# agussomacal/ROMHighContrast

Hardware: AMD Instinct MI355X
Metric: snapshot_solves_per_sec (higher is better)
Workload: dtype f64

## Files before the change

romhighcontrast_amd/csrc/rom_fem_kernels.hip:

```cpp
#include "rom_fem_dev.h"

__global__ void k_build_A0(double* A0, const double* Qp, const double* rho, int n1, int n1p, int N) {
  size_t idx = blockIdx.x * size_t(blockDim.x) + threadIdx.x;
  size_t total = size_t(n1) * n1 * n1p;
  if (idx >= total) return;
  int m = int(idx % n1p);
  size_t ij = idx / n1p;
  int j = int(ij % n1) + 1, i = int(ij / n1) + 1;
  A0[idx] = (m < n1) ? Qp[size_t(j - 1) * n1p + m] * rho[size_t(m) * (N + 1) + i] : 0.0;
}

__global__ void k_repack_table(const double* __restrict__ G, int ld, int nseg, int n1, int orient, double* __restrict__ Gs) {
  const long long idx = blockIdx.x * (long long)blockDim.x + threadIdx.x;
  const long long hrows = (long long)n1 * n1;
  if (idx >= (long long)nseg * hrows * 8) return;
  const int kk = int(idx & 7);
  const long long rp = (idx >> 3) % hrows, seg = (idx >> 3) / hrows;
  const long long row = orient ? (rp % n1) * n1 + rp / n1 : rp;
  const int k = int(seg) * 8 + kk;
  Gs[idx] = k < ld ? G[row * ld + k] : 0.0;
}

__global__ void k_mask_table(double* __restrict__ G, int ld, int n1, ExtThresholds th) {
  const long long idx = blockIdx.x * (long long)blockDim.x + threadIdx.x;
// ... 442 lines not shown
  for (int i = threadIdx.x; i < f.nsc; i += blockDim.x) {
    const int b0 = f.scb[2 * i], b1 = f.scb[2 * i + 1];
    y[f.spos0 + i] = b1 >= 0 ? 1.0 / (am[b0] + am[b1]) : (1.0 / (double(f.N) * double(f.N))) / am[b0];
  }
  for (int task = threadIdx.x; task < f.nctask; task += blockDim.x) {
    const int4 t0 = reinterpret_cast<const int4*>(f.ctask)[2 * task], t1 = reinterpret_cast<const int4*>(f.ctask)[2 * task + 1];
    const int len = t0.z, ldm = t0.w;
    const double* Mt = f.cm + t0.x;
    const double* src = ys + t0.y;
    double dot = 0.0;
#pragma unroll 16
    for (int j = 0; j < len; ++j) dot += Mt[size_t(j) * ldm] * src[j];
    if (t1.x >= 0) dot += f.vec[t1.x] / (am[t1.y] + am[t1.z]);
    dots[t1.w] = dot;
  }
  __syncthreads();
  for (int it = threadIdx.x; it < f.ncoef; it += blockDim.x) {
    const CoefGroup& cg = f.groups[f.item_group[it]];
    const int k = f.item_k[it];
    const double s = am[cg.b0] + am[cg.b1];
    double out = 0.0;
    if (k == cg.r) {
      out = 1.0 / s;
    } else if (k < cg.r) {
      if (cg.kind == 0) {
        out = ys[cg.zpos + k];
      } else {
        const double* dk = dots + size_t(f.item_cf[it]) * 8;
        double acc = 0.0;
        for (int t = 0; t < cg.nterm; ++t) acc += (cg.t[t].blk >= 0 ? am[cg.t[t].blk] : s / 2) * dk[t];
        out = acc / s;
      }
    }
    y[cg.cpos + k] = out;
  }
}

__global__ __launch_bounds__(256) void k_expand(FemDev f, const double* __restrict__ a, int Mc, double* __restrict__ U,
                                                long long row0) {
  __shared__ __align__(16) double lds[STAGE_TOTAL];
  expand_tile(f, Mc, U, row0, lds, blockIdx.x, blockIdx.y, blockIdx.z);
}

__global__ __launch_bounds__(256) void k_back_pre(FemDev f, const double* __restrict__ a, int Mc) {
  __shared__ __align__(16) double lds[STAGE_TOTAL];
  const WavePos wp;
  const PreEdge& pe = f.pre[blockIdx.z];
  const int srow = stage_row(), sseg = stage_seg();
  const int mA = blockIdx.y * 64 + srow;
  const int iB = blockIdx.x * 64 + srow;
  const double* am = mA < Mc ? a + size_t(mA) * f.kblk : nullptr;
  const double seA = am ? am[pe.e0] + am[pe.e1] : 0.0;
  Acc acc;
  acc_zero(acc);
  for (int q = 0; q < pe.nnb; ++q) {
    const PreNb nb = pe.nb[q];
    const double* pA = am ? f.y + size_t(mA) * f.nGp + nb.fpos + sseg : nullptr;
    const double* pB = f.Bt + (size_t(nb.bt) * f.n1p + iB) * f.n1p + sseg;
    const double cu = !am ? 0.0 : (nb.blk >= 0 ? am[nb.blk] : seA / 2);
    gemm_loop(
        nb.nch,
        [&](int ch, double* v) {
          load4_aligned(pA ? pA + ch * BK : nullptr, v);
#pragma unroll
          for (int x = 0; x < 4; ++x) v[x] *= cu;
        },
        [&](int ch, double* v) { load4_aligned(pB + ch * BK, v); }, acc, lds, wp);
  }
#pragma unroll
  for (int i = 0; i < 2; ++i)
#pragma unroll
    for (int g = 0; g < 4; ++g) {
      const int m = blockIdx.y * 64 + acc_row(wp, i, g);
      if (m >= Mc) continue;
      const double* amr = a + size_t(m) * f.kblk;
      const double inv = 1.0 / (amr[pe.e0] + amr[pe.e1]);
#pragma unroll
      for (int jb = 0; jb < 2; ++jb) {
        const int node = blockIdx.x * 64 + acc_col(wp, jb);
        f.y[size_t(m) * f.nGp + pe.pos + node] = node < f.n1 ? (f.vec[pe.woff + node] + acc.c[i][jb][g]) * inv : 0.0;
      }
    }
}

template <int NS>
__device__ inline void diag_update_body(const FemDev& f, const double* __restrict__ am0, int m0, int nsys, int slot, double* lds,
                                        double* coef) {
  const WavePos wp;
  const TileDesc& d = f.desc[slot];
  const bool lower = !(wp.wr == 0 && wp.wc == 1);
  if (f.tile_stream && d.t1 - d.t0 <= 128) {
    TileStream<NS> ts;
    s_tile_stream_begin<NS>(ts, slot, d, f, am0, nsys);
    SymAcc acc[NS];
#pragma unroll
    for (int q = 0; q < NS; ++q) {
      sym_acc_zero(acc[q]);
      if (q >= nsys) continue;
      if (q > 0) __syncthreads();
      accumulate_klist_dma<true>(f, slot, f.L + size_t(m0 + q) * f.nslots * 4096, [](int) { return true; }, acc[q], reinterpret_cast<char*>(lds), wp);
    }
    __syncthreads();
    double* T[NS];
#pragma unroll
    for (int q = 0; q < NS; ++q) T[q] = lds + q * TILE_DOUBLES;
    s_tile_to_lds<NS>(T, ts, d, f);
#pragma unroll
    for (int q = 0; q < NS; ++q) {
      if (q >= nsys) break;
      tile_minus_acc_sym(T[q], acc[q], wp);
      double* Lout = f.L + (size_t(m0 + q) * f.nslots + slot) * 4096;
      for (int idx = threadIdx.x; idx < 4096; idx += 256) Lout[idx] = T[q][(idx >> 6) * LDC + (idx & 63)];
    }
    return;
  }
  double* Cb = lds;
  STile st[NS];
  s_tile_load<NS>(st, d, f, am0, nsys, coef);
#pragma unroll
  for (int q = 0; q < NS; ++q) {
    if (q >= nsys) break;
    double* Lm = f.L + size_t(m0 + q) * f.nslots * 4096;
    Acc acc;
    acc_zero(acc);
    if (q > 0) __syncthreads();
    accumulate_klist_dma(f, slot, Lm, [&](int) { return lower; }, acc, reinterpret_cast<char*>(lds), wp);
    tile_from_acc(Cb, acc, st[q], wp);
    double* Lout = Lm + size_t(slot) * 4096;
    for (int idx = threadIdx.x; idx < 4096; idx += 256) Lout[idx] = Cb[(idx >> 6) * LDC + (idx & 63)];
  }
}
template <int NS>
__global__ __launch_bounds__(256, NS == 1 ? 4 : 2) void k_diag_update(FemDev f, const double* __restrict__ a, int slot, int Mc) {
  __shared__ __align__(16) double lds[NS * TILE_DOUBLES];
  __shared__ double coef[NS * COEF_MAX + TERM_DESC_DOUBLES];
  static_assert(TD_LDS_BYTES <= TILE_DOUBLES * 8, "the DMA slots fit under the tile");
  const int m0 = blockIdx.x * NS;
  diag_update_body<NS>(f, a + size_t(m0) * f.kblk, m0, min(NS, Mc - m0), slot, lds, coef);
}
template __global__ void k_diag_update<1>(FemDev, const double*, int, int);
template __global__ void k_diag_update<2>(FemDev, const double*, int, int);

__device__ inline double rsqrt_newton(double d) {
  double y = __builtin_amdgcn_rsq(d);
  const double hd = 0.5 * d;
  y = y * fma(-hd * y, y, 1.5);
  y = y * fma(-hd * y, y, 1.5);
  return y;
}


__device__ __host__ constexpr int s1_lrow(int r) { return 8 * (r >> 2) * ((r >> 2) + 1) + (r & 3) * 4 * ((r >> 2) + 1); }

__device__ inline bool chol_pivots_bad(double myrs) {
  return __builtin_amdgcn_ballot_w64(!(myrs > 0.0 && myrs < 1.0e300)) != 0;
}
__device__ inline void chol_panel_core(int lane, int c0, double (&v)[4], double& y, double& myrs, double a00, double a10,
                                       double a11, double a20, double a21, double a22, double a30, double a31, double a32, double a33) {
  const double y0 = readlane_f64(y, c0);
  double y1 = readlane_f64(y, c0 + 1), y2 = readlane_f64(y, c0 + 2), y3 = readlane_f64(y, c0 + 3);
  const double rs0 = rsqrt_newton(a00);
  const double l10 = a10 * rs0, l20 = a20 * rs0, l30 = a30 * rs0;
  a11 -= l10 * l10; a21 -= l20 * l10; a31 -= l30 * l10;
  a22 -= l20 * l20; a32 -= l30 * l20; a33 -= l30 * l30;
  const double yd0 = y0 * rs0;
  y1 -= l10 * yd0; y2 -= l20 * yd0; y3 -= l30 * yd0;
  {
    const double l = lane >= c0 ? v[0] * rs0 : 0.0;
    v[0] = l;
    if (lane == c0) {
      y = yd0;
      myrs = rs0;
    } else if (lane > c0) {
      y -= l * yd0;
    }
    v[1] -= l * l10; v[2] -= l * l20; v[3] -= l * l30;
  }
  const double rs1 = rsqrt_newton(a11);
  const double l21 = a21 * rs1, l31 = a31 * rs1;
  a22 -= l21 * l21; a32 -= l31 * l21; a33 -= l31 * l31;
  const double yd1 = y1 * rs1;
  y2 -= l21 * yd1; y3 -= l31 * yd1;
  {
    const double l = lane >= c0 + 1 ? v[1] * rs1 : 0.0;
    v[1] = l;
    if (lane == c0 + 1) {
      y = yd1;
      myrs = rs1;
    } else if (lane > c0 + 1) {
      y -= l * yd1;
    }
    v[2] -= l * l21; v[3] -= l * l31;
  }
  const double rs2 = rsqrt_newton(a22);
  const double l32 = a32 * rs2;
  a33 -= l32 * l32;
  const double yd2 = y2 * rs2;
  y3 -= l32 * yd2;
  {
    const double l = lane >= c0 + 2 ? v[2] * rs2 : 0.0;
    v[2] = l;
    if (lane == c0 + 2) {
      y = yd2;
      myrs = rs2;
    } else if (lane > c0 + 2) {
      y -= l * yd2;
    }
    v[3] -= l * l32;
  }
  const double rs3 = rsqrt_newton(a33);
  const double yd3 = y3 * rs3;
  {
    const double l = lane >= c0 + 3 ? v[3] * rs3 : 0.0;
    v[3] = l;
    if (lane == c0 + 3) {
      y = yd3;
      myrs = rs3;
    } else if (lane > c0 + 3) {
      y -= l * yd3;
    }
  }
}
__device__ inline void chol_panel_rows(const double* Pn, int lane, int c0, double (&v)[4], double& y, double& myrs) {
  {
    const double2 v01 = *reinterpret_cast<const double2*>(&Pn[lane * 4]);
    const double2 v23 = *reinterpret_cast<const double2*>(&Pn[lane * 4 + 2]);
    v[0] = v01.x; v[1] = v01.y; v[2] = v23.x; v[3] = v23.y;
  }
  const double a00 = Pn[c0 * 4];
  const double2 r1 = *reinterpret_cast<const double2*>(&Pn[(c0 + 1) * 4]);
  const double2 r2 = *reinterpret_cast<const double2*>(&Pn[(c0 + 2) * 4]);
  const double a22 = Pn[(c0 + 2) * 4 + 2];
  const double2 r3a = *reinterpret_cast<const double2*>(&Pn[(c0 + 3) * 4]);
  const double2 r3b = *reinterpret_cast<const double2*>(&Pn[(c0 + 3) * 4 + 2]);
  chol_panel_core(lane, c0, v, y, myrs, a00, r1.x, r1.y, r2.x, r2.y, a22, r3a.x, r3a.y, r3b.x, r3b.y);
}
__device__ inline void chol_panel_regs(int lane, int c0, double (&v)[4], double& y, double& myrs) {
  chol_panel_core(lane, c0, v, y, myrs, readlane_f64(v[0], c0), readlane_f64(v[0], c0 + 1), readlane_f64(v[1], c0 + 1),
                  readlane_f64(v[0], c0 + 2), readlane_f64(v[1], c0 + 2), readlane_f64(v[2], c0 + 2), readlane_f64(v[0], c0 + 3),
                  readlane_f64(v[1], c0 + 3), readlane_f64(v[2], c0 + 3), readlane_f64(v[3], c0 + 3));
}

__device__ inline void tile_rows_to_global(double* __restrict__ dst, const double* Ls, int lane) {
  for (int i = 0; i < 64; ++i) dst[i * 64 + lane] = Ls[i * LDC + lane];
}

#ifdef ROMHC_DIAGF_STAMPS
#define DF_STAMP(i) df_stamp[i] = __builtin_readcyclecounter()
#else
#define DF_STAMP(i)
#endif
__device__ inline void diag_factor_body(const FemDev& f, int m, int slot, int j, double* Ls, double* Pn, double* rinv) {
#ifdef ROMHC_DIAGF_STAMPS
  unsigned long long df_stamp[8];
#endif
  DF_STAMP(0);
  const int lane = threadIdx.x & 63;
  const int l16 = lane & 15, l4 = lane >> 4;
  double* Lt = f.L + (size_t(m) * f.nslots + slot) * 4096;
  d4_t C[4][4];
#pragma unroll
  for (int ib = 0; ib < 4; ++ib)
#pragma unroll
    for (int jb = 0; jb <= ib; ++jb)
#pragma unroll
      for (int g = 0; g < 4; ++g) {
        const int R = 16 * ib + 4 * g + l4, Cc = 16 * jb + l16;
        C[ib][jb][g] = Lt[max(R, Cc) * 64 + min(R, Cc)];
      }
  double y = f.y[size_t(m) * f.nGp + j * 64 + lane];
  double myrs = 0.0;
#ifdef ROMHC_DIAGF_STAMPS
  asm volatile("s_waitcnt vmcnt(0)" ::: "memory");
#endif
  DF_STAMP(1);
#pragma unroll
  for (int p = 0; p < 16; ++p) {
    const int jb = p >> 2, co = 4 * (p & 3), c0 = 4 * p;
    if ((l16 >> 2) == (p & 3)) {
#pragma unroll
      for (int ib = jb; ib < 4; ++ib)
#pragma unroll
        for (int g = 0; g < 4; ++g) Pn[(16 * ib + 4 * g + l4) * 4 + (l16 - co)] = C[ib][jb][g];
    }
    __builtin_amdgcn_wave_barrier();
    double v[4];
    chol_panel_rows(Pn, lane, c0, v, y, myrs);
    __builtin_amdgcn_wave_barrier();
    *reinterpret_cast<double2*>(&Pn[lane * 4]) = double2{v[0], v[1]};
    *reinterpret_cast<double2*>(&Pn[lane * 4 + 2]) = double2{v[2], v[3]};
    *reinterpret_cast<double2*>(&Ls[lane * LDC + c0]) = double2{v[0], v[1]};
    *reinterpret_cast<double2*>(&Ls[lane * LDC + c0 + 2]) = double2{v[2], v[3]};
    __builtin_amdgcn_wave_barrier();
    if (p < 15) {
      double frag[4];
#pragma unroll
      for (int x = jb; x < 4; ++x) frag[x] = Pn[(16 * x + l16) * 4 + l4];
#pragma unroll
      for (int jb2 = jb; jb2 < 4; ++jb2)
#pragma unroll
        for (int ib = jb2; ib < 4; ++ib)
          C[ib][jb2] = __builtin_amdgcn_mfma_f64_16x16x4f64(-frag[ib], frag[jb2], C[ib][jb2], 0, 0, 0);
    }
    __builtin_amdgcn_wave_barrier();
  }
  DF_STAMP(2);
  if (chol_pivots_bad(myrs) && lane == 0) atomicOr(f.status, 1);
  f.y[size_t(m) * f.nGp + j * 64 + lane] = y;
  rinv[lane] = myrs;
  __builtin_amdgcn_wave_barrier();
  tile_rows_to_global(Lt, Ls, lane);
  DF_STAMP(3);
  {
    const int bi = lane >> 4, r = lane & 15;
    const double* Lb = Ls + (16 * bi) * LDC + 16 * bi;
    double xr[16];
#pragma unroll
    for (int c = 15; c >= 0; --c) {
      double lc[16];
#pragma unroll
      for (int k = c + 1; k < 16; ++k) lc[k] = Lb[k * LDC + c];
      double s0 = 0.0, s1 = 0.0;
#pragma unroll
      for (int k = c + 1; k < 16; k += 2) {
        s0 = __builtin_fma(xr[k], lc[k], s0);
        if (k + 1 < 16) s1 = __builtin_fma(xr[k + 1], lc[k + 1], s1);
      }
      const double rc = rinv[16 * bi + c];
      xr[c] = r == c ? rc : (r > c ? -rc * (s0 + s1) : 0.0);
    }
    __builtin_amdgcn_wave_barrier();
#pragma unroll
    for (int c = 0; c < 16; c += 2) *reinterpret_cast<double2*>(&Ls[lane * LDC + 16 * bi + c]) = double2{xr[c], xr[c + 1]};
    __builtin_amdgcn_wave_barrier();
  }
  DF_STAMP(4);
#pragma unroll
  for (int jb = 2; jb >= 0; --jb) {
    d4_t W[4];
#pragma unroll
    for (int ib = jb + 1; ib < 4; ++ib) {
      W[ib] = d4_t{0.0, 0.0, 0.0, 0.0};
#pragma unroll
      for (int kk = 0; kk < 16; kk += 4) {
        const double af = Ls[(16 * ib + l16) * LDC + 16 * jb + kk + l4];
        const double bf = Ls[(16 * jb + kk + l4) * LDC + 16 * jb + l16];
        W[ib] = __builtin_amdgcn_mfma_f64_16x16x4f64(af, bf, W[ib], 0, 0, 0);
      }
    }
    __builtin_amdgcn_wave_barrier();
#pragma unroll
    for (int ib = jb + 1; ib < 4; ++ib)
#pragma unroll
      for (int g = 0; g < 4; ++g) Ls[(16 * ib + 4 * g + l4) * LDC + 16 * jb + l16] = W[ib][g];
    __builtin_amdgcn_wave_barrier();
    d4_t X[4];
#pragma unroll
    for (int ib = jb + 1; ib < 4; ++ib) {
      X[ib] = d4_t{0.0, 0.0, 0.0, 0.0};
#pragma unroll
      for (int kb = jb + 1; kb <= ib; ++kb)
#pragma unroll
        for (int kk = 0; kk < 16; kk += 4) {
          const double af = Ls[(16 * ib + l16) * LDC + 16 * kb + kk + l4];
          const double bf = Ls[(16 * kb + kk + l4) * LDC + 16 * jb + l16];
          X[ib] = __builtin_amdgcn_mfma_f64_16x16x4f64(-af, bf, X[ib], 0, 0, 0);
        }
    }
    __builtin_amdgcn_wave_barrier();
#pragma unroll
    for (int ib = jb + 1; ib < 4; ++ib)
#pragma unroll
      for (int g = 0; g < 4; ++g) Ls[(16 * ib + 4 * g + l4) * LDC + 16 * jb + l16] = X[ib][g];
    __builtin_amdgcn_wave_barrier();
  }
  __builtin_amdgcn_wave_barrier();
  DF_STAMP(5);
  double* It = f.invL + (size_t(m) * f.T + j) * 4096;
  tile_rows_to_global(It, Ls, lane);
  DF_STAMP(6);
#ifdef ROMHC_DIAGF_STAMPS
  asm volatile("s_waitcnt vmcnt(0)" ::: "memory");
  DF_STAMP(7);
  if (lane == 0 && (m == 0 || m == 513))
    printf("diagf m %d j %d: load %llu panels %llu store_L %llu inv_diag %llu inv_offdiag %llu store_X_issue %llu store_X_drain %llu total %llu\n", m, j,
           df_stamp[1] - df_stamp[0], df_stamp[2] - df_stamp[1], df_stamp[3] - df_stamp[2], df_stamp[4] - df_stamp[3],
           df_stamp[5] - df_stamp[4], df_stamp[6] - df_stamp[5], df_stamp[7] - df_stamp[6], df_stamp[7] - df_stamp[0]);
#endif
}
#undef DF_STAMP
constexpr int DIAGF_LDS_DOUBLES = 64 * LDC + 64 * 4 + 64;
__global__ __launch_bounds__(64) void k_diag_factor(FemDev f, int slot, int j) {
  __shared__ __align__(16) double lds[DIAGF_LDS_DOUBLES];
  diag_factor_body(f, blockIdx.x, slot, j, lds, lds + 64 * LDC, lds + 64 * LDC + 256);
}


__global__ __launch_bounds__(512) void k_solve1(FemDev f, const double* __restrict__ a, int Mc) {
  extern __shared__ __align__(16) char s1_dyn[];
  const int w8 = __builtin_amdgcn_readfirstlane(int(threadIdx.x) >> 6), w = w8 & 3, lane = threadIdx.x & 63;
  const bool upd = w8 >= 4;
  double* const coefs = reinterpret_cast<double*>(s1_dyn);
  const double* const Dl = reinterpret_cast<const double*>(s1_dyn + S1_COEF_BYTES + 4 * S1_WAVE_BYTES);
  double* const Ls = reinterpret_cast<double*>(s1_dyn + S1_COEF_BYTES + w * S1_WAVE_BYTES);
  double* const Pn = Ls + 40 * 64;
  double* const zs = Pn + 64 * 4;
  double* const aL = zs + 64;
  double* const Pn1 = aL + 64;
  double* const PnB = Pn1 + 64 * 4;
  double* const wz = Ls;
  static_assert(DENSE_GROUPS_MAX * 64 <= 40 * 64 && 8 * 16 * 17 <= 40 * 64, "the shared area holds each of its three tenants");
  static_assert(S1_WAVE_BYTES == (40 * 64 + 64 * 4 + 64 + 64 + 3 * 64 * 4) * 8 && S1_COEF_BYTES == 4 * 64 * 8, "LDS areas");
  const int m_raw = 4 * int(blockIdx.x) + w;
  const bool live = m_raw < Mc;
  const int m = live ? m_raw : Mc - 1;
  const double* am = a + size_t(m) * f.kblk;
  double* ym = f.y + size_t(m) * f.nGp;
#ifdef ROMHC_SOLVE1_STAMPS
  unsigned long long stamp[10];
#define S1_STAMP(i) stamp[i] = __builtin_readcyclecounter()
  S1_STAMP(0);
#else
#define S1_STAMP(i)
#endif
#define S1_WAVE_SYNC()                                   \
  do {                                                   \
    asm volatile("s_waitcnt lgkmcnt(0)" ::: "memory");   \
    __builtin_amdgcn_wave_barrier();                     \
  } while (0)
#define S1_BARRIER() asm volatile("s_waitcnt lgkmcnt(0)\n\ts_barrier" ::: "memory")
  const int l16 = lane & 15, l4 = lane >> 4;

  if (upd) {
    int4 irec[6], crec[S1_ITEM_PASSES];
    int wd[DENSE_GROUPS_MAX];
    {
      const int4* ir = reinterpret_cast<const int4*>(f.s1_items) + size_t(min(lane, max(f.ndi, 1) - 1)) * 6;
#pragma unroll
      for (int x = 0; x < 6; ++x) irec[x] = ir[x];
#pragma unroll
      for (int r = 0; r < S1_ITEM_PASSES; ++r) crec[r] = reinterpret_cast<const int4*>(f.s1_citems)[min(lane + 64 * r, max(f.ncoef, 1) - 1)];
#pragma unroll
      for (int g = 0; g < DENSE_GROUPS_MAX; ++g) wd[g] = g < f.ndg ? f.dweight[g * 64 + lane] : -2;
    }
    const int xr_first = lane < f.ncross ? f.xred[lane] : 0;
    const int2 sc_b = lane < f.nsc ? reinterpret_cast<const int2*>(f.scb)[lane] : int2{0, 0};
    const RhsTerm rt = f.rhs[min(lane, max(f.nrhs, 1) - 1)];
    const double gvec = f.g[lane];
    __syncthreads();
    {
      const double rcoef = lane < f.nrhs ? (rt.kind == 0 ? aL[rt.b0] / (aL[rt.e0] + aL[rt.e1]) : 0.5) : 0.0;
      double y = gvec;
      for (int t0 = 0; t0 < f.nrhs; t0 += 8) {
        double rv[8];
#pragma unroll
        for (int x = 0; x < 8; ++x) {
          rv[x] = 0.0;
          if (t0 + x < f.nrhs) {
            const int pos = __builtin_amdgcn_readlane(rt.pos, t0 + x), len = __builtin_amdgcn_readlane(rt.len, t0 + x);
            const int voff = __builtin_amdgcn_readlane(rt.voff, t0 + x);
            if (lane >= pos && lane < pos + len) rv[x] = f.vec[voff + lane - pos];
          }
// ... 80 lines not shown
            for (int g = 0; g < 4; ++g) dstp[(16 * ib + 4 * g + l4) * 4 + (l16 - co1)] = C[ib][jb1][g];
        }
      }
#ifdef ROMHC_SOLVE1_PANEL_STAMPS
      { const unsigned long long t0_ = __builtin_readcyclecounter(); S1_BARRIER(); uwait += __builtin_readcyclecounter() - t0_; }
#else
      S1_BARRIER();
#endif
      const double* Pp = (p & 1) ? Pn1 : Pn;
      double frag[4];
#pragma unroll
      for (int x = jb; x < 4; ++x) frag[x] = Pp[(16 * x + l16) * 4 + l4];
#pragma unroll
      for (int jb2 = jb; jb2 < 4; ++jb2)
#pragma unroll
        for (int ib = jb2; ib < 4; ++ib)
          C[ib][jb2] = __builtin_amdgcn_mfma_f64_16x16x4f64(-frag[ib], frag[jb2], C[ib][jb2], 0, 0, 0);
    }
#ifdef ROMHC_SOLVE1_PANEL_STAMPS
    const unsigned long long ut1 = __builtin_readcyclecounter();
#endif
    S1_BARRIER();
    if (!live) return;
    const double z = zs[lane];
    ym[lane] = z;
    if (lane < f.ncross) ym[f.xb0 + lane] = zs[xr_first];
    for (int x = lane + 64; x < f.ncross; x += 64) ym[f.xb0 + x] = zs[f.xred[x]];
#pragma unroll
    for (int g = 0; g < DENSE_GROUPS_MAX; ++g)
      if (g < f.ndg) wz[g * 64 + lane] = wgt[g] * z;
    S1_WAVE_SYNC();
    if (has_it) {
      const double* wg = wz + it_g * 64;
      const double* D = Dl + lane;
      double acc = 0.0;
#pragma unroll 1
      for (int j0 = 0; j0 < 64; j0 += 16) {
#pragma unroll
        for (int j = 0; j < 16; ++j) acc += D[(j0 + j) * f.ndi] * wg[j0 + j];
      }
#pragma unroll
      for (int v = 0; v < 4; ++v)
        if (v < it_nv) acc += it_cv[v] * it_vv[v];
      ym[it_pos] = acc / it_den;
    }
#pragma unroll
    for (int r = 0; r < S1_ITEM_PASSES; ++r)
      if (ci_src[r] >= 0) ym[ci_dst[r]] = zs[ci_src[r]];
    for (int it = lane + 64 * S1_ITEM_PASSES; it < f.ncoef; it += 64) {
      const CoefGroup& cg = f.groups[f.item_group[it]];
      const int k = f.item_k[it];
      if (cg.kind == 1 && k < cg.r) continue;
      ym[cg.cpos + k] = k == cg.r ? 1.0 / (aL[cg.b0] + aL[cg.b1]) : (k < cg.r ? zs[cg.zpos + k] : 0.0);
    }
#ifdef ROMHC_SOLVE1_STAMPS
    if (lane < 12) ym[lane] = PnB[lane];
#ifdef ROMHC_SOLVE1_PANEL_STAMPS
    if (lane == 12) ym[12] = double(uwait);
    if (lane == 13) ym[13] = double(ut1 - ut0);
#endif
#endif
    return;
  }

  {
    const unsigned d0 = unsigned(size_t((__attribute__((address_space(3))) char*)s1_dyn)) + unsigned(S1_COEF_BYTES + 4 * S1_WAVE_BYTES);
    const int nchunk = (f.ndi + 1) >> 1;
    const char* src = reinterpret_cast<const char*>(f.dmat);
    for (int c = w; c < nchunk; c += 4)
      asm volatile("s_mov_b32 m0, %0\n\tglobal_load_lds_dwordx4 %1, %2" ::"s"(__builtin_amdgcn_readfirstlane(d0 + unsigned(c) * 1024u)),
                   "v"(unsigned(lane) * 16u), "s"(x128_uniform(src + size_t(c) * 1024))
                   : "memory", "m0");
  }
  {
    const int p0 = f.wp0[w], np = f.wp0[w + 1] - p0;
    const double2* pbase = reinterpret_cast<const double2*>(f.pool_acc) + size_t(p0) * 128 + lane;
    double2 v[PAIR_RING][2];
    auto issue = [&](int i, double2 (&dst)[2]) {
      dst[0] = pbase[size_t(i) * 128];
      dst[1] = pbase[size_t(i) * 128 + 64];
    };
    const double a_l = lane < f.kblk ? am[lane] : 1.0;
    const GenTerm gt = f.terms[f.s1_t0 + min(lane, f.s1_nterm - 1)];
    int mine = f.wmeta[p0 + lane];
#pragma unroll
    for (int u = 0; u < PAIR_RING; ++u) issue(u, v[u]);
#pragma unroll
    for (int x = 0; x < 40; ++x) Ls[x * 64 + lane] = 0.0;
    aL[lane] = a_l;
    S1_WAVE_SYNC();
    coefs[w * 64 + lane] = lane < f.s1_nterm ? term_coef(gt, aL) : 0.0;
    __syncthreads();
    double cf[4];
#pragma unroll
    for (int s = 0; s < 4; ++s) cf[s] = coefs[s * 64 + lane];
    double acc4[4][4];
#pragma unroll
    for (int s = 0; s < 4; ++s)
#pragma unroll
      for (int g = 0; g < 4; ++g) acc4[s][g] = 0.0;
    double* const Cl0 = reinterpret_cast<double*>(s1_dyn + S1_COEF_BYTES) + lane;
    S1_STAMP(1);
    for (int base = 0; base < np; base += 64) {
      const int cur = mine;
      const int nxt = f.wmeta[p0 + base + 64 + lane];
      const int cnt = min(64, np - base);
#pragma unroll
      for (int i0 = 0; i0 < 64; i0 += PAIR_RING) {
        if (i0 >= cnt) break;
#pragma unroll
        for (int u = 0; u < PAIR_RING; ++u) {
          const int i = i0 + u;
          const int meta = __builtin_amdgcn_readlane(cur, i);
#pragma unroll
          for (int s = 0; s < 4; ++s) {
            const double c = readlane_f64(cf[s], meta & 0xff);
            acc4[s][0] = __builtin_fma(c, v[u][0].x, acc4[s][0]);
            acc4[s][1] = __builtin_fma(c, v[u][0].y, acc4[s][1]);
            acc4[s][2] = __builtin_fma(c, v[u][1].x, acc4[s][2]);
            acc4[s][3] = __builtin_fma(c, v[u][1].y, acc4[s][3]);
          }
          if (meta >> 16) {
            double* dst = Cl0 + ((meta >> 8) & 0xff) * 256;
#pragma unroll
            for (int s = 0; s < 4; ++s)
#pragma unroll
              for (int g = 0; g < 4; ++g) {
                dst[s * (S1_WAVE_BYTES / 8) + g * 64] = acc4[s][g];
                acc4[s][g] = 0.0;
              }
          }
          issue(base + i + PAIR_RING, v[u]);
        }
      }
      mine = nxt;
    }
    asm volatile("s_waitcnt vmcnt(0)" ::: "memory");
    __syncthreads();
  }
  S1_STAMP(2);
  double nv[4];
  {
    const int ib = lane >> 4;
    const double* src = Ls + ((ib * (ib + 1) / 2) * 4 + ((lane >> 2) & 3)) * 64 + (lane & 3) * 16;
    const double2 x0 = *reinterpret_cast<const double2*>(src), x1 = *reinterpret_cast<const double2*>(src + 2);
    nv[0] = x0.x; nv[1] = x0.y; nv[2] = x1.x; nv[3] = x1.y;
#pragma unroll
    for (int k = 0; k < 4; ++k)
      if (lane >= f.s1_ndr || k >= f.s1_ndr) nv[k] = lane == k ? 1.0 : 0.0;
  }
  S1_BARRIER();
  S1_STAMP(3);
  double y = zs[lane];
  double myrs = 0.0;
#ifdef ROMHC_SOLVE1_PANEL_STAMPS
  unsigned long long fwait = 0;
#endif
  S1_STAMP(4);
#pragma unroll
  for (int p = 0; p < 16; ++p) {
    const int c0 = 4 * p;
    chol_panel_regs(lane, c0, nv, y, myrs);
    {
      double* Pp = (p & 1) ? Pn1 : Pn;
      *reinterpret_cast<double2*>(&Pp[lane * 4]) = double2{nv[0], nv[1]};
      *reinterpret_cast<double2*>(&Pp[lane * 4 + 2]) = double2{nv[2], nv[3]};
    }
    if ((lane >> 2) >= p) {
      double* lrow = Ls + s1_lrow(lane) + c0;
      *reinterpret_cast<double2*>(lrow) = double2{nv[0], nv[1]};
      *reinterpret_cast<double2*>(lrow + 2) = double2{nv[2], nv[3]};
    }
    if (p < 15) {
#ifdef ROMHC_SOLVE1_PANEL_STAMPS
      { const unsigned long long t0_ = __builtin_readcyclecounter(); S1_BARRIER(); fwait += __builtin_readcyclecounter() - t0_; }
#else
      S1_BARRIER();
#endif
      const double* bp = PnB + ((p + 1) & 1) * 256 + lane * 4;
      const double2 b01 = *reinterpret_cast<const double2*>(bp), b23 = *reinterpret_cast<const double2*>(bp + 2);
      double nn[4] = {b01.x, b01.y, b23.x, b23.y};
#pragma unroll
      for (int kk = 0; kk < 4; ++kk)
#pragma unroll
        for (int k = 0; k < 4; ++k) nn[kk] = __builtin_fma(-nv[k], readlane_f64(nv[k], c0 + 4 + kk), nn[kk]);
#pragma unroll
      for (int kk = 0; kk < 4; ++kk) nv[kk] = nn[kk];
    }
  }
  if (chol_pivots_bad(myrs) && live && lane == 0) atomicOr(f.status, 1);
  S1_WAVE_SYNC();
  S1_STAMP(5);
#pragma unroll
  for (int h = 1; h >= 0; --h) {
    double lcol[32];
#pragma unroll
    for (int j = 0; j < 32; ++j) lcol[j] = Ls[s1_lrow(32 * h + j) + lane];
#pragma unroll
    for (int j = 31; j >= 0; --j) {
      const int jj = 32 * h + j;
      const double xj = readlane_f64(y, jj) * readlane_f64(myrs, jj);
      if (lane == jj) y = xj;
      else if (lane < jj) y -= lcol[j] * xj;
    }
  }
  zs[lane] = y;
  S1_STAMP(6);
#ifdef ROMHC_SOLVE1_STAMPS
#pragma unroll
  for (int k = 0; k < 7; ++k)
    if (lane == k) PnB[k] = double(stamp[k] - stamp[0]);
  if (lane >= 7 && lane < 12) PnB[lane] = 0.0;
#ifdef ROMHC_SOLVE1_PANEL_STAMPS
  if (lane == 10) PnB[10] = double(fwait);
#endif
#endif
  S1_BARRIER();
#undef S1_STAMP
#undef S1_WAVE_SYNC
#undef S1_BARRIER
}

template <int NS>
__device__ inline void panel_body(const FemDev& f, const double* __restrict__ am0, int m0, int nsys, int j, int ent, double* lds,
                                  double* yj, double* coef) {
  double* Cb = lds;
  double* stB = lds + TILE_DOUBLES;
  const int slot = f.colrow[ent];
  const int ti = f.colti[ent];
  const WavePos wp;
  const TileDesc& d = f.desc[slot];
  const int t = threadIdx.x;
  const bool stream = NS == 1 && f.tile_stream && d.t1 - d.t0 <= 128;
  STile st[NS];
  if (!stream) s_tile_load<NS>(st, d, f, am0, nsys, coef);
  static_assert(TD_LDS_BYTES <= FACT_LDS_DOUBLES * 8, "the DMA slots alias the staging area and the C tile");
#pragma unroll
  for (int q = 0; q < NS; ++q) {
    if (q >= nsys) break;
    const int m = m0 + q;
    double* Lm = f.L + size_t(m) * f.nslots * 4096;
    if (q > 0) __syncthreads();
    if (t < 64) yj[t] = f.y[size_t(m) * f.nGp + j * 64 + t];
    TileStream<1> ts;
    if (stream) s_tile_stream_begin<1>(ts, slot, d, f, am0 + size_t(q) * f.kblk, 1);
    Acc acc;
    acc_zero(acc);
    accumulate_klist_dma(f, slot, Lm, [](int) { return true; }, acc, reinterpret_cast<char*>(lds), wp);
    if (stream) {
      __syncthreads();
      double* T[1] = {Cb};
      s_tile_to_lds<1>(T, ts, d, f);
      tile_minus_acc(Cb, acc, wp);
    } else {
      tile_from_acc(Cb, acc, st[q], wp);
    }

    acc_zero(acc);
    const double* I = f.invL + (size_t(m) * f.T + j) * 4096 + (t >> 2) * 64 + (t & 3) * 2;
    const int kmax = (wp.wc + 1) * 32;
    {
      const int fr = wp.lane & 15, kq = wp.lane >> 4;
      double2 vb = *reinterpret_cast<const double2*>(I);
      for (int ch = 0; ch < 8; ++ch) {
        *reinterpret_cast<double2*>(stB + (t >> 2) * LDK8 + (t & 3) * 2) = vb;
        __syncthreads();
        if (ch + 1 < 8) vb = *reinterpret_cast<const double2*>(I + (ch + 1) * 8);
        if (ch * 8 < kmax) {
          const double* pa = Cb + (wp.wr * 32 + fr) * LDC + ch * 8 + kq;
          const double* pb = stB + (wp.wc * 32 + fr) * LDK8 + kq;
#pragma unroll
          for (int kk = 0; kk < 8; kk += 4) {
            const double a0 = pa[kk], a1 = pa[16 * LDC + kk];
            const double b0 = pb[kk], b1 = pb[16 * LDK8 + kk];
            acc.c[0][0] = __builtin_amdgcn_mfma_f64_16x16x4f64(a0, b0, acc.c[0][0], 0, 0, 0);
            acc.c[0][1] = __builtin_amdgcn_mfma_f64_16x16x4f64(a0, b1, acc.c[0][1], 0, 0, 0);
            acc.c[1][0] = __builtin_amdgcn_mfma_f64_16x16x4f64(a1, b0, acc.c[1][0], 0, 0, 0);
            acc.c[1][1] = __builtin_amdgcn_mfma_f64_16x16x4f64(a1, b1, acc.c[1][1], 0, 0, 0);
          }
        }
        __syncthreads();
      }
    }

    double* Lout = Lm + size_t(slot) * 4096;
#pragma unroll
    for (int i = 0; i < 2; ++i)
#pragma unroll
      for (int jb = 0; jb < 2; ++jb)
#pragma unroll
        for (int g = 0; g < 4; ++g) {
          int r = acc_row(wp, i, g), c = acc_col(wp, jb);
          double v = acc.c[i][jb][g];
          Lout[r * 64 + c] = v;
          Cb[r * LDC + c] = v;
        }
    __syncthreads();
    if (t < 64) {
      double sum = 0.0;
      for (int k = 0; k < 64; ++k) sum += Cb[t * LDC + k] * yj[k];
      f.y[size_t(m) * f.nGp + ti * 64 + t] -= sum;
    }
  }
}

__device__ inline void panel_block(int b, int nrows, int Mc, int& m, int& row) {
  const int xcd = b & 7, idx = b >> 3;
  const int full = (Mc >> 3) << 3;
  m = xcd + 8 * (idx / nrows);
  row = idx % nrows;
  if (m >= full) {
    const int tb = b - full * nrows;
    m = full + tb / nrows;
    row = tb % nrows;
  }
}

template <int NS>
__global__ __launch_bounds__(256, 4) void k_factor_panel(FemDev f, const double* __restrict__ a, int j, int Mc) {
  __shared__ __align__(16) double lds[FACT_LDS_DOUBLES];
  __shared__ double yj[64];
  double* coef = lds;
  int mp, row;
  panel_block(blockIdx.x, f.colptr[j + 1] - f.colptr[j], (Mc + NS - 1) / NS, mp, row);
  const int m0 = mp * NS;
  panel_body<NS>(f, a + size_t(m0) * f.kblk, m0, min(NS, Mc - m0), j, f.colptr[j] + row, lds, yj, coef);
}
template __global__ void k_factor_panel<1>(FemDev, const double*, int, int);

__global__ __launch_bounds__(256) void k_backsolve(FemDev f) {
  extern __shared__ __align__(16) double xs[];
  __shared__ double red[4][64];
  __shared__ double vs[64];
  const int m = blockIdx.x;
  const int t = threadIdx.x, c = t & 63, part = t >> 6;
  const double* Lm = f.L + size_t(m) * f.nslots * 4096;
  double* ym = f.y + size_t(m) * f.nGp;
  for (int j = f.T - 1; j >= 0; --j) {
    double s = 0.0;
    for (int e = f.colptr[j]; e < f.colptr[j + 1]; ++e) {
      const double* Lt = Lm + size_t(f.colrow[e]) * 4096;
      const double* xi = xs + f.colti[e] * 64;
#pragma unroll 4
      for (int rr = part * 16; rr < part * 16 + 16; ++rr) s += Lt[rr * 64 + c] * xi[rr];
    }
    red[part][c] = s;
    __syncthreads();
    if (t < 64) vs[t] = ym[j * 64 + t] - (red[0][t] + red[1][t] + red[2][t] + red[3][t]);
    __syncthreads();
    const double* It = f.invL + (size_t(m) * f.T + j) * 4096;
    s = 0.0;
#pragma unroll 4
    for (int rr = part * 16; rr < part * 16 + 16; ++rr) s += It[rr * 64 + c] * vs[rr];
    red[part][c] = s;
    __syncthreads();
    if (t < 64) xs[j * 64 + t] = red[0][t] + red[1][t] + red[2][t] + red[3][t];
    __syncthreads();
  }
  for (int v = t; v < f.nGa; v += 256) ym[v] = xs[v];
// ... 453 lines not shown
```

Before: 4.443 million.

## Block the back-substitution by 4x4 diagonal blocks and park pivots in LDS

Pivot reciprocal square roots are now written to LDS as each panel of four is finished, instead of being held in a per-lane register and gathered with readlane. The solve_1 back-substitution is rewritten to walk 4x4 diagonal blocks. The next block's triangle and column entries are prefetched from LDS, and the four unknowns of a block are computed from scalar-broadcast values, which should shorten the serial readlane dependency chain compared with 64 one-column steps. The divergent y update branches become fma plus select. The cost is extra LDS traffic and a large register array (tri[16][10], lc[16][4]) that may raise register pressure.

```diff
diff --git a/romhighcontrast_amd/csrc/rom_fem_kernels.hip b/romhighcontrast_amd/csrc/rom_fem_kernels.hip
--- a/romhighcontrast_amd/csrc/rom_fem_kernels.hip
+++ b/romhighcontrast_amd/csrc/rom_fem_kernels.hip
@@ -618,10 +618,14 @@
 
 __device__ __host__ constexpr int s1_lrow(int r) { return 8 * (r >> 2) * ((r >> 2) + 1) + (r & 3) * 4 * ((r >> 2) + 1); }
 
+__device__ inline void chol_park_rs(double* dst, const double (&rs)[4]) {
+  *reinterpret_cast<double2*>(dst) = double2{rs[0], rs[1]};
+  *reinterpret_cast<double2*>(dst + 2) = double2{rs[2], rs[3]};
+}
 __device__ inline bool chol_pivots_bad(double myrs) {
   return __builtin_amdgcn_ballot_w64(!(myrs > 0.0 && myrs < 1.0e300)) != 0;
 }
-__device__ inline void chol_panel_core(int lane, int c0, double (&v)[4], double& y, double& myrs, double a00, double a10,
+__device__ inline void chol_panel_core(int lane, int c0, double (&v)[4], double& y, double (&rs)[4], double a00, double a10,
                                        double a11, double a20, double a21, double a22, double a30, double a31, double a32, double a33) {
   const double y0 = readlane_f64(y, c0);
   double y1 = readlane_f64(y, c0 + 1), y2 = readlane_f64(y, c0 + 2), y3 = readlane_f64(y, c0 + 3);
@@ -634,12 +638,8 @@
   {
     const double l = lane >= c0 ? v[0] * rs0 : 0.0;
     v[0] = l;
-    if (lane == c0) {
-      y = yd0;
-      myrs = rs0;
-    } else if (lane > c0) {
-      y -= l * yd0;
-    }
+    const double yu = __builtin_fma(-l, yd0, y);
+    y = lane == c0 ? yd0 : (lane > c0 ? yu : y);
     v[1] -= l * l10; v[2] -= l * l20; v[3] -= l * l30;
   }
   const double rs1 = rsqrt_newton(a11);
@@ -650,12 +650,8 @@
   {
     const double l = lane >= c0 + 1 ? v[1] * rs1 : 0.0;
     v[1] = l;
-    if (lane == c0 + 1) {
-      y = yd1;
-      myrs = rs1;
-    } else if (lane > c0 + 1) {
-      y -= l * yd1;
-    }
+    const double yu = __builtin_fma(-l, yd1, y);
+    y = lane == c0 + 1 ? yd1 : (lane > c0 + 1 ? yu : y);
     v[2] -= l * l21; v[3] -= l * l31;
   }
   const double rs2 = rsqrt_newton(a22);
@@ -666,12 +662,8 @@
   {
     const double l = lane >= c0 + 2 ? v[2] * rs2 : 0.0;
     v[2] = l;
-    if (lane == c0 + 2) {
-      y = yd2;
-      myrs = rs2;
-    } else if (lane > c0 + 2) {
-      y -= l * yd2;
-    }
+    const double yu = __builtin_fma(-l, yd2, y);
+    y = lane == c0 + 2 ? yd2 : (lane > c0 + 2 ? yu : y);
     v[3] -= l * l32;
   }
   const double rs3 = rsqrt_newton(a33);
@@ -679,15 +671,12 @@
   {
     const double l = lane >= c0 + 3 ? v[3] * rs3 : 0.0;
     v[3] = l;
-    if (lane == c0 + 3) {
-      y = yd3;
-      myrs = rs3;
-    } else if (lane > c0 + 3) {
-      y -= l * yd3;
-    }
-  }
-}
-__device__ inline void chol_panel_rows(const double* Pn, int lane, int c0, double (&v)[4], double& y, double& myrs) {
+    const double yu = __builtin_fma(-l, yd3, y);
+    y = lane == c0 + 3 ? yd3 : (lane > c0 + 3 ? yu : y);
+  }
+  rs[0] = rs0; rs[1] = rs1; rs[2] = rs2; rs[3] = rs3;
+}
+__device__ inline void chol_panel_rows(const double* Pn, int lane, int c0, double (&v)[4], double& y, double (&rs)[4]) {
   {
     const double2 v01 = *reinterpret_cast<const double2*>(&Pn[lane * 4]);
     const double2 v23 = *reinterpret_cast<const double2*>(&Pn[lane * 4 + 2]);
@@ -699,10 +688,10 @@
   const double a22 = Pn[(c0 + 2) * 4 + 2];
   const double2 r3a = *reinterpret_cast<const double2*>(&Pn[(c0 + 3) * 4]);
   const double2 r3b = *reinterpret_cast<const double2*>(&Pn[(c0 + 3) * 4 + 2]);
-  chol_panel_core(lane, c0, v, y, myrs, a00, r1.x, r1.y, r2.x, r2.y, a22, r3a.x, r3a.y, r3b.x, r3b.y);
-}
-__device__ inline void chol_panel_regs(int lane, int c0, double (&v)[4], double& y, double& myrs) {
-  chol_panel_core(lane, c0, v, y, myrs, readlane_f64(v[0], c0), readlane_f64(v[0], c0 + 1), readlane_f64(v[1], c0 + 1),
+  chol_panel_core(lane, c0, v, y, rs, a00, r1.x, r1.y, r2.x, r2.y, a22, r3a.x, r3a.y, r3b.x, r3b.y);
+}
+__device__ inline void chol_panel_regs(int lane, int c0, double (&v)[4], double& y, double (&rs)[4]) {
+  chol_panel_core(lane, c0, v, y, rs, readlane_f64(v[0], c0), readlane_f64(v[0], c0 + 1), readlane_f64(v[1], c0 + 1),
                   readlane_f64(v[0], c0 + 2), readlane_f64(v[1], c0 + 2), readlane_f64(v[2], c0 + 2), readlane_f64(v[0], c0 + 3),
                   readlane_f64(v[1], c0 + 3), readlane_f64(v[2], c0 + 3), readlane_f64(v[3], c0 + 3));
 }
@@ -735,7 +724,6 @@
         C[ib][jb][g] = Lt[max(R, Cc) * 64 + min(R, Cc)];
       }
   double y = f.y[size_t(m) * f.nGp + j * 64 + lane];
-  double myrs = 0.0;
 #ifdef ROMHC_DIAGF_STAMPS
   asm volatile("s_waitcnt vmcnt(0)" ::: "memory");
 #endif
@@ -750,8 +738,9 @@
         for (int g = 0; g < 4; ++g) Pn[(16 * ib + 4 * g + l4) * 4 + (l16 - co)] = C[ib][jb][g];
     }
     __builtin_amdgcn_wave_barrier();
-    double v[4];
-    chol_panel_rows(Pn, lane, c0, v, y, myrs);
+    double v[4], rs[4];
+    chol_panel_rows(Pn, lane, c0, v, y, rs);
+    chol_park_rs(rinv + c0, rs);
     __builtin_amdgcn_wave_barrier();
     *reinterpret_cast<double2*>(&Pn[lane * 4]) = double2{v[0], v[1]};
     *reinterpret_cast<double2*>(&Pn[lane * 4 + 2]) = double2{v[2], v[3]};
@@ -771,9 +760,8 @@
     __builtin_amdgcn_wave_barrier();
   }
   DF_STAMP(2);
-  if (chol_pivots_bad(myrs) && lane == 0) atomicOr(f.status, 1);
+  if (chol_pivots_bad(rinv[lane]) && lane == 0) atomicOr(f.status, 1);
   f.y[size_t(m) * f.nGp + j * 64 + lane] = y;
-  rinv[lane] = myrs;
   __builtin_amdgcn_wave_barrier();
   tile_rows_to_global(Lt, Ls, lane);
   DF_STAMP(3);
@@ -1160,7 +1148,6 @@
   S1_BARRIER();
   S1_STAMP(3);
   double y = zs[lane];
-  double myrs = 0.0;
 #ifdef ROMHC_SOLVE1_PANEL_STAMPS
   unsigned long long fwait = 0;
 #endif
@@ -1168,7 +1155,9 @@
 #pragma unroll
   for (int p = 0; p < 16; ++p) {
     const int c0 = 4 * p;
-    chol_panel_regs(lane, c0, nv, y, myrs);
+    double rs[4];
+    chol_panel_regs(lane, c0, nv, y, rs);
+    chol_park_rs(zs + c0, rs);
     {
       double* Pp = (p & 1) ? Pn1 : Pn;
       *reinterpret_cast<double2*>(&Pp[lane * 4]) = double2{nv[0], nv[1]};
@@ -1196,23 +1185,48 @@
       for (int kk = 0; kk < 4; ++kk) nv[kk] = nn[kk];
     }
   }
-  if (chol_pivots_bad(myrs) && live && lane == 0) atomicOr(f.status, 1);
   S1_WAVE_SYNC();
+  if (chol_pivots_bad(zs[lane]) && live && lane == 0) atomicOr(f.status, 1);
   S1_STAMP(5);
-#pragma unroll
-  for (int h = 1; h >= 0; --h) {
-    double lcol[32];
-#pragma unroll
-    for (int j = 0; j < 32; ++j) lcol[j] = Ls[s1_lrow(32 * h + j) + lane];
-#pragma unroll
-    for (int j = 31; j >= 0; --j) {
-      const int jj = 32 * h + j;
-      const double xj = readlane_f64(y, jj) * readlane_f64(myrs, jj);
-      if (lane == jj) y = xj;
-      else if (lane < jj) y -= lcol[j] * xj;
-    }
-  }
-  zs[lane] = y;
+  {
+    double tri[16][10];
+    double lc[16][4];
+    auto fetch_block = [&](int q) {
+      const int b = 4 * q;
+      const double2 r1 = *reinterpret_cast<const double2*>(&Ls[s1_lrow(b + 1) + b]);
+      const double2 r2 = *reinterpret_cast<const double2*>(&Ls[s1_lrow(b + 2) + b]);
+      const double2 r3 = *reinterpret_cast<const double2*>(&Ls[s1_lrow(b + 3) + b]);
+      const double l32 = Ls[s1_lrow(b + 3) + b + 2];
+      const double2 s01 = *reinterpret_cast<const double2*>(&zs[b]), s23 = *reinterpret_cast<const double2*>(&zs[b + 2]);
+      double (&t)[10] = tri[q];
+      t[0] = r1.x; t[1] = r2.x; t[2] = r2.y; t[3] = r3.x; t[4] = r3.y; t[5] = l32;
+      t[6] = s01.x; t[7] = s01.y; t[8] = s23.x; t[9] = s23.y;
+#pragma unroll
+      for (int i = 0; i < 4; ++i) lc[q][i] = Ls[s1_lrow(b + i) + lane];
+    };
+    fetch_block(15);
+    const bool odd = lane & 1, upper = lane & 2;
+    double u = y;
+    double x = 0.0;
+#pragma unroll
+    for (int q = 15; q >= 0; --q) {
+      if (q >= 1) fetch_block(q - 1);
+      const double (&t)[10] = tri[q];
+      const double y0 = readlane_f64(u, 4 * q), y1 = readlane_f64(u, 4 * q + 1), y2 = readlane_f64(u, 4 * q + 2), y3 = readlane_f64(u, 4 * q + 3);
+      const double x3 = y3 * t[9];
+      u = __builtin_fma(-lc[q][3], x3, u);
+      const double x2 = __builtin_fma(-t[5], x3, y2) * t[8];
+      u = __builtin_fma(-lc[q][2], x2, u);
+      const double x1 = __builtin_fma(-t[2], x2, __builtin_fma(-t[4], x3, y1)) * t[7];
+      u = __builtin_fma(-lc[q][1], x1, u);
+      const double x0 = __builtin_fma(-t[0], x1, __builtin_fma(-t[1], x2, __builtin_fma(-t[3], x3, y0))) * t[6];
+      u = __builtin_fma(-lc[q][0], x0, u);
+      const double xhi = odd ? x3 : x2, xlo = odd ? x1 : x0;
+      const double xs = upper ? xhi : xlo;
+      x = (lane >> 2) == q ? xs : x;
+    }
+    zs[lane] = x;
+  }
   S1_STAMP(6);
 #ifdef ROMHC_SOLVE1_STAMPS
 #pragma unroll
```

After: 4.502 million (median of 6 runs). 1.01x the previous value.
